# NevVerVer/DBS-Gym

Measured on AMD Instinct MI355X. Metric: env steps/sec (whole node), N=1024 osc x 4096 envs per GPU, higher is better.
Workload: dtype f32 (bf16x3-split products, f32 accumulate)

## Files before the change

### dbs-gym_amd/abi.py

```python
from __future__ import annotations

import ctypes
import os
from ctypes import POINTER, c_double, c_float, c_int, c_int32, c_int64, c_uint8, c_void_p

KURA_ABI_VERSION = 2
KURA_S_MAX = 32
KURA_MAX_BINS = 32
KURA_NSTATS = 8

KURA_F_MAX_STEPS = 1
KURA_F_NONFINITE = 2
KURA_F_GRID = 8
KURA_F_BARRIER = 16
KURA_F_BOUNDS = 32
FLAG_NAMES = {
    KURA_F_MAX_STEPS: "The maximum number of solver steps was reached",
    KURA_F_NONFINITE: "non-finite (NaN/Inf) state or RHS",
    KURA_F_GRID: "save grid outside [2, KURA_S_MAX] samples",
    KURA_F_BARRIER: "split-group barrier timed out",
    KURA_F_BOUNDS: "device access outside its buffer (KURA_DEBUG build)",
}

KURA_REC_NAIVE = 0
# ... 79 lines not shown
    "kura_create": (c_int, [POINTER(KuraConfig), c_int, POINTER(c_void_p)]),
    "kura_destroy": (c_int, [c_void_p]),
    "kura_last_error": (ctypes.c_char_p, []),
    "kura_abi_version": (c_int, []),
    "kura_set_coupling": (c_int, [c_void_p, c_void_p]),
    "kura_set_env_params": (c_int, [c_void_p, c_int, c_int, c_void_p, c_void_p, c_void_p]),
    "kura_set_spectral": (c_int, [c_void_p, c_void_p, c_void_p]),
    "kura_reset": (c_int, [c_void_p, c_void_p, c_void_p, c_void_p, c_void_p]),
    "kura_step": (c_int, [c_void_p, c_void_p, c_void_p, c_void_p, c_void_p, c_void_p, c_void_p, c_void_p,
                          c_void_p]),
    "kura_reward": (c_int, [c_void_p, c_int, c_void_p, c_void_p, c_void_p, c_int, c_void_p]),
    "kura_reward_n": (c_int, [c_void_p, c_int, c_void_p, c_int64, c_int64, c_int, c_void_p, c_void_p, c_int,
                              c_void_p, c_void_p, c_void_p]),
    "kura_get_state": (c_int, [c_void_p, c_void_p, c_void_p, c_void_p, c_void_p, c_void_p]),
    "kura_set_state": (c_int, [c_void_p, c_void_p, c_void_p, c_void_p, c_void_p, c_void_p]),
    "kura_get_spec": (c_int, [c_void_p, c_void_p]),
    "kura_set_spec": (c_int, [c_void_p, c_void_p]),
    "kura_set_env_gain": (c_int, [c_void_p, c_int, c_int, c_void_p]),
    "kura_psd_bbpow": (c_int, [c_void_p, c_void_p, c_void_p, c_int64, c_int, c_double, c_double, c_double, c_void_p,
                               c_void_p]),
    "kura_episode_bbpow": (c_int, [c_void_p, c_void_p, c_double, c_double, c_double, c_void_p, c_void_p]),
    "kura_envelope_stats": (c_int, [c_void_p, c_void_p, c_void_p, c_int64, c_int, c_void_p, c_void_p]),
    "kura_episode_envelope_stats": (c_int, [c_void_p, c_void_p, c_void_p, c_void_p]),
    "kura_get_stats": (c_int, [c_void_p, c_void_p, c_int]),
    "kura_get_env_flags": (c_int, [c_void_p, c_void_p, c_void_p]),
    "kura_set_row_capture": (c_int, [c_void_p, c_void_p]),
    "kura_set_transient_capture": (c_int, [c_void_p, c_void_p]),
    "kura_set_transient_rows": (c_int, [c_void_p, c_void_p]),
    "kura_transient_len": (c_int, [c_void_p]),
    "kura_get_stamps": (c_int, [c_void_p, c_void_p]),
    "kura_selftest_math": (c_int, [c_void_p, c_void_p, c_void_p, c_int]),
    "kura_selftest_gemm": (c_int, [c_void_p, c_void_p, c_void_p, c_int]),
    "kura_selftest_coupling": (c_int, [c_void_p, c_void_p, c_void_p, c_int, c_int]),
}

PKG_DIR = os.path.dirname(os.path.abspath(__file__))
LIB_PATH = os.path.join(PKG_DIR, "csrc", "libkura.so")

_lib = None


def load_library(path: str | None = None) -> ctypes.CDLL:
    global _lib
    if _lib is not None and path is None:
        return _lib
    p = path or os.environ.get("KURA_LIB") or LIB_PATH
    if not os.path.exists(p):
        raise RuntimeError(
            f"libkura.so not found at {p}: build it with `python -c 'import __graft_entry__ as g; g.build()'` "
            "(the HIP library is the only implementation of the step path; there is no CPU fallback)")
    lib = ctypes.CDLL(p)
    for name, (res, args) in _SYMBOLS.items():
        fn = getattr(lib, name)
        fn.restype = res
        fn.argtypes = args
    for name, (res, args) in _DEBUG_SYMBOLS.items():
        if hasattr(lib, name):
            fn = getattr(lib, name)
            fn.restype = res
            fn.argtypes = args
    if lib.kura_abi_version() != KURA_ABI_VERSION:
        raise RuntimeError("libkura ABI version mismatch")
    if path is None:
        _lib = lib
    return lib

# ... 38 lines not shown
```

### dbs-gym_amd/csrc/kura_capi.inc

```
#include <stdarg.h>
#include <stdlib.h>
#include <stdio.h>
#include <string.h>

#include <algorithm>
#include <string>
#include <unordered_map>
#include <utility>
#include <vector>

#include "kura_r2.h"

namespace {

thread_local char g_err[512] = "";

int set_err(int code, const char* fmt, ...) {
    va_list ap;
    va_start(ap, fmt);
    vsnprintf(g_err, sizeof(g_err), fmt, ap);
    va_end(ap);
    return code;
}

// ... 101 lines not shown

static void fill_params(KuraHandle* h) {
    const KuraConfig& c = h->cfg;
    DevParams& p = h->p;
    p.N = c.n_osc;
    p.B = c.n_envs;
    p.W = c.window;
    p.n_elec = c.n_elec;
    p.n_rec = c.n_rec;
    p.rec_kernel = c.rec_kernel;
    p.reward_kind = c.reward_kind;
    p.episode_steps = c.episode_steps;
    p.max_steps = c.max_steps;
    p.n_bins = c.n_bins;
    p.padlen = c.padlen;
    for (int i = 0; i < KURA_MAX_BINS; ++i) p.bins[i] = c.bins[i];
    p.dt = c.dt;
    p.width = c.width;
    p.pause = c.pause;
    p.transient_len = c.transient_len;
    p.act_lo = c.act_lo;
    p.act_hi = c.act_hi;
    p.dbs_lo = c.dbs_lo;
    p.dbs_hi = c.dbs_hi;
    for (int i = 0; i < 5; ++i) { p.bw_b[i] = c.bw_b[i]; p.bw_a[i] = c.bw_a[i]; }
    for (int i = 0; i < 4; ++i) p.bw_zi[i] = c.bw_zi[i];
    p.rtol = c.rtol;
    p.atol = c.atol;
    p.kn = c.kn;
    p.dt0 = c.dt0;
    p.alpha_sw = h->alpha_sw;
    p.alpha_dd = h->alpha_dd;
    p.alpha_dd_bytes = (unsigned)(h->alpha_dd_cap * sizeof(float));
    p.omega = h->omega;
    p.kn_env = h->kn_env;
    p.g_stim = h->g_stim;
    p.g_rec = h->g_rec;
    p.ctab = h->ctab;
    p.stab = h->stab;
    p.y = h->y;
    p.t = h->t;
    p.step = h->step;
    p.ring = h->ring;
    p.wpos = h->wpos;
    p.R = h->R;
    p.pulse = h->pulse;
    p.r2c = h->r2c;
    p.spec = h->spec;
    p.stats = h->stats;
    p.stamps = h->stamps;
    p.npart = h->xl ? c.n_osc / (h->tpw * 256) : 1;
    p.npairs = h->ngroups * p.npart;
    p.xg = h->xg;
    p.xred = h->xred;
    p.xredd = h->xredd;
    p.gcnt = h->gcnt;
    p.episode_cap = c.episode_cap;
    p.ep_lfp = h->ep_lfp;
    p.ep_len = h->ep_len;
    p.eflags = h->eflags;
    p.rows = nullptr;
    p.lfp_tr = nullptr;
    p.rows_tr = nullptr;
    p.n_tr = (int)ceil((c.transient_len - 0.0) / c.dt);
    p.gemm_dump = nullptr;
    p.gemm_dump_n = 0;
// ... 12 lines not shown
}

static uint16_t bf16_rne(float f) {
    uint32_t u;
    memcpy(&u, &f, 4);
    return (uint16_t)((u + 0x7fffu + ((u >> 16) & 1u)) >> 16);
}
static float bf16_f(uint16_t h) {
    const uint32_t u = (uint32_t)h << 16;
    float f;
    memcpy(&f, &u, 4);
    return f;
}
static void split_fragment(const float* alpha, int N, int jt, int b, uint16_t* f) {
    for (int lane = 0; lane < 64; ++lane)
        for (int i = 0; i < 8; ++i) {
            const int col = 32 * jt + (lane & 31);
            const int k = 16 * b + 8 * (i / 4) + 2 * (i % 4) + (lane >> 5);
            const float a = alpha[(size_t)col * N + k];
            const uint16_t h1 = bf16_rne(a);
            const float r1 = a - bf16_f(h1);
            const uint16_t h2 = bf16_rne(r1);
            const uint16_t h3 = bf16_rne(r1 - bf16_f(h2));
            const uint16_t hp[3] = {h1, h2, h3};
            for (int p = 0; p < 3; ++p) f[(p * 64 + lane) * 8 + i] = hp[p];
        }
}
static void split_alpha(const float* alpha, uint16_t* sp, int N) {
    const int NB = N / 16;
    for (int jt = 0; jt < N / 32; ++jt)
        for (int b = 0; b < NB; ++b) split_fragment(alpha, N, jt, b, sp + ((size_t)jt * NB + b) * 3 * 64 * 8);
}

static bool presplit_image(int N, bool sp, int tpw) {
    return sp && (N <= XL_NL || tpw > KURA_XL_SP_STAGED_MAXTPW);
}
static uint64_t fnv1a64(const void* p, size_t n) {
    const unsigned char* c = static_cast<const unsigned char*>(p);
    uint64_t h = 1469598103934665603ull;
    for (size_t i = 0; i < n; ++i) h = (h ^ c[i]) * 1099511628211ull;
    return h;
}
static std::vector<float> split_alpha_dedup(const float* alpha, int N, int* nfrag = nullptr) {
    const int NB = N / 16, NT = N / 32;
    const size_t FU16 = 3 * 64 * 8;
    const size_t MAPF = (size_t)NT * NB;
    std::vector<uint16_t> frags;
    std::vector<int32_t> map(MAPF);
    std::unordered_multimap<uint64_t, int> seen;
    std::vector<uint16_t> f(FU16);
    int n = 0;
    for (int jt = 0; jt < NT; ++jt)
        for (int b = 0; b < NB; ++b) {
            split_fragment(alpha, N, jt, b, f.data());
            const uint64_t key = fnv1a64(f.data(), FU16 * 2);
            int id = -1;
            for (auto r = seen.equal_range(key); r.first != r.second; ++r.first)
                if (!memcmp(frags.data() + (size_t)r.first->second * FU16, f.data(), FU16 * 2)) {
                    id = r.first->second;
                    break;
                }
            if (id < 0) {
                id = n++;
                seen.emplace(key, id);
                frags.insert(frags.end(), f.begin(), f.end());
            }
// ... 203 lines not shown
                    nb < 1)
                    rc = set_err(KURA_E_UNSUPPORTED, "split-group kernel does not fit a CU (occupancy %d)", nb);
            }
        }
    }
    if (rc) {
        int keep = rc;
        kura_destroy(h);
        return keep;
    }
    fill_params(h);
    *out = h;
    return KURA_OK;
}

int kura_destroy(KuraHandle* h) {
    if (!h) return KURA_OK;
    (void)hipSetDevice(h->device);
    void* ptrs[] = {h->alpha_sw, h->alpha_dd, h->omega, h->kn_env, h->g_stim, h->g_rec, h->ctab, h->stab, h->y, h->t, h->step,
                    h->ring, h->wpos, h->R, h->pulse, h->r2c, h->spec, h->stats, h->stamps,
                    h->xg, h->xred, h->xredd, h->gcnt, h->ep_lfp, h->ep_len, h->met_scratch,
                    h->eflags};
    for (void* q : ptrs)
        if (q) (void)hipFree(q);
    for (auto& kv : h->r2c_len) (void)hipFree(kv.second);
    delete h;
    return KURA_OK;
}

int kura_set_coupling(KuraHandle* h, const float* alpha) {
    if (!h || !alpha) return set_err(KURA_E_INVALID, "null argument");
    HIP_TRY(hipSetDevice(h->device));
    const int N = h->cfg.n_osc;
    const std::vector<float> sw = coupling_image(alpha, N, h->sp, h->tpw);
    if (sw.size() > h->alpha_cap) {
        HIP_TRY(hipDeviceSynchronize());
        HIP_TRY(hipFree(h->alpha_sw));
        h->alpha_sw = nullptr;
        h->alpha_cap = 0;
        if (int rc = dalloc(&h->alpha_sw, sw.size())) return rc;
        h->alpha_cap = sw.size();
        h->p.alpha_sw = h->alpha_sw;
    }
    HIP_TRY(hipMemcpy(h->alpha_sw, sw.data(), sw.size() * sizeof(float), hipMemcpyHostToDevice));
    if (h->sp && !h->xl) {
        const std::vector<float> dd = split_alpha_dedup(alpha, N);
        if (dd.size() > h->alpha_dd_cap) {
            HIP_TRY(hipDeviceSynchronize());
            if (h->alpha_dd) HIP_TRY(hipFree(h->alpha_dd));
            h->alpha_dd = nullptr;
            h->alpha_dd_cap = 0;
            if (int rc = dalloc(&h->alpha_dd, dd.size())) return rc;
            h->alpha_dd_cap = dd.size();
            h->p.alpha_dd = h->alpha_dd;
            h->p.alpha_dd_bytes = (unsigned)(dd.size() * sizeof(float));
        }
        HIP_TRY(hipMemcpy(h->alpha_dd, dd.data(), dd.size() * sizeof(float), hipMemcpyHostToDevice));
    }
    h->have_coupling = true;
    return KURA_OK;
}

int kura_set_env_params(KuraHandle* h, int env0, int n, const float* omega, const double* g_stim,
                        const double* g_rec) {
    if (!h) return set_err(KURA_E_INVALID, "null handle");
    if (env0 < 0 || n < 0 || env0 + n > h->B) return set_err(KURA_E_INVALID, "env range [%d,%d) outside [0,%d)", env0, env0 + n, h->B);
    HIP_TRY(hipSetDevice(h->device));
    const size_t N = h->cfg.n_osc;
    if (omega)
        HIP_TRY(hipMemcpy(h->omega + (size_t)env0 * N, omega, (size_t)n * N * sizeof(float), hipMemcpyHostToDevice));
    if (g_stim)
        HIP_TRY(hipMemcpy(h->g_stim + (size_t)env0 * h->cfg.n_elec * N, g_stim,
                          (size_t)n * h->cfg.n_elec * N * sizeof(double), hipMemcpyHostToDevice));
    if (g_rec && h->cfg.n_rec > 0) {
        std::vector<double> G((size_t)n * N);
        const int nr = h->cfg.n_rec;
        for (int b = 0; b < n; ++b)
            for (size_t i = 0; i < N; ++i) {
                double acc = g_rec[((size_t)b * nr) * N + i];
                for (int r = 1; r < nr; ++r) acc = acc + g_rec[((size_t)b * nr + r) * N + i];
                G[(size_t)b * N + i] = acc;
            }
        HIP_TRY(hipMemcpy(h->g_rec + (size_t)env0 * N, G.data(), G.size() * sizeof(double), hipMemcpyHostToDevice));
    }
    if (omega && g_stim) h->have_params = true;
    return KURA_OK;
}

int kura_set_env_gain(KuraHandle* h, int env0, int n, const float* kn) {
    if (!h || !kn) return set_err(KURA_E_INVALID, "null argument");
    if (env0 < 0 || n < 0 || env0 + n > h->B) return set_err(KURA_E_INVALID, "env range [%d,%d) outside [0,%d)", env0, env0 + n, h->B);
    for (int b = 0; b < n; ++b)
        if (!(kn[b] == kn[b])) return set_err(KURA_E_INVALID, "kn[%d] is nan", env0 + b);
// ... 401 lines not shown
    for (int i = 0; i < n && i < KURA_NSTATS; ++i) out[i] = (int64_t)v[i];
    return KURA_OK;
}

int kura_get_stamps(KuraHandle* h, uint64_t* out ) {
    if (!h || !out) return set_err(KURA_E_INVALID, "null argument");
    HIP_TRY(hipSetDevice(h->device));
    HIP_TRY(hipDeviceSynchronize());
    HIP_TRY(hipMemcpy(out, h->stamps, NWAVES * KURA_NSTAMP * sizeof(uint64_t), hipMemcpyDeviceToHost));
    HIP_TRY(hipMemset(h->stamps, 0, NWAVES * KURA_NSTAMP * sizeof(uint64_t)));
    return KURA_OK;
}

int kura_selftest_math(const float* x, const float* y, float* out, int n) {
    if (n <= 0 || !x || !y || !out) return set_err(KURA_E_INVALID, "bad args");
    float *dx = nullptr, *dy = nullptr, *dout = nullptr;
    int rc = dalloc(&dx, n);
    rc = rc ? rc : dalloc(&dy, n);
    rc = rc ? rc : dalloc(&dout, (size_t)n * KURA_SELFTEST_MATH_W);
    if (!rc) {
        (void)hipMemcpy(dx, x, n * sizeof(float), hipMemcpyHostToDevice);
        (void)hipMemcpy(dy, y, n * sizeof(float), hipMemcpyHostToDevice);
        hipLaunchKernelGGL(kura_selftest_math_kernel, dim3((n + 255) / 256), dim3(256), 0, 0, dx, dy, dout, n);
        hipError_t e = hipDeviceSynchronize();
        if (e != hipSuccess) rc = set_err(KURA_E_HIP, "selftest_math: %s", hipGetErrorString(e));
        else (void)hipMemcpy(out, dout, (size_t)n * KURA_SELFTEST_MATH_W * sizeof(float), hipMemcpyDeviceToHost);
    }
    (void)hipFree(dx);
    (void)hipFree(dy);
    (void)hipFree(dout);
    return rc;
}

int kura_selftest_coupling(const float* X , const float* alpha , float* Y , int N,
                           int coupling) {
    if (N != 256 && N != 512 && N != 1024) return set_err(KURA_E_UNSUPPORTED, "N=%d", N);
    if (coupling != KURA_COUPLING_AUTO && coupling != KURA_COUPLING_F32 && coupling != KURA_COUPLING_BF16X3)
        return set_err(KURA_E_INVALID, "coupling=%d", coupling);
    const bool sp = coupling != KURA_COUPLING_F32;
    const std::vector<float> sw = coupling_image(alpha, N, sp, N / 256);
    float *dX = nullptr, *dA = nullptr, *dY = nullptr;
    int rc = dalloc(&dX, (size_t)32 * N);
    rc = rc ? rc : dalloc(&dA, sw.size());
    rc = rc ? rc : dalloc(&dY, (size_t)32 * N);
    const size_t lds = (size_t)xs_floats(N) * sizeof(float);
    const void* k = selftest_gemm_kernel(N / 256, sp);
    if (!rc && hipFuncSetAttribute(k, hipFuncAttributeMaxDynamicSharedMemorySize, (int)lds) != hipSuccess)
        rc = set_err(KURA_E_HIP, "selftest_gemm: LDS attribute");
    if (!rc) {
        (void)hipMemcpy(dX, X, (size_t)32 * N * sizeof(float), hipMemcpyHostToDevice);
        (void)hipMemcpy(dA, sw.data(), sw.size() * sizeof(float), hipMemcpyHostToDevice);
        void* argv[] = {(void*)&dX, (void*)&dA, (void*)&dY, (void*)&N};
        hipError_t e = hipLaunchKernel(k, dim3(1), dim3(NTHREADS), argv, lds, 0);
        if (e == hipSuccess) e = hipDeviceSynchronize();
        if (e != hipSuccess) rc = set_err(KURA_E_HIP, "selftest_gemm: %s", hipGetErrorString(e));
        else (void)hipMemcpy(Y, dY, (size_t)32 * N * sizeof(float), hipMemcpyDeviceToHost);
    }
    (void)hipFree(dX);
    (void)hipFree(dA);
    (void)hipFree(dY);
    return rc;
}

int kura_selftest_gemm(const float* X, const float* alpha, float* Y, int N) {
    return kura_selftest_coupling(X, alpha, Y, N, KURA_COUPLING_F32);
}

}
```

### dbs-gym_amd/csrc/kura_kernels.hip

```cpp
#include <hip/hip_runtime.h>
#include <stdint.h>

#include "../../include/kura.h"
#include "kura_detmath.h"

#pragma clang fp contract(off)

#define E_WG 16
#define NWAVES 8
#define NTHREADS (NWAVES * 64)
#define ENVS_PER_WAVE (E_WG / NWAVES)

typedef float floatx4 __attribute__((ext_vector_type(4)));
typedef float floatx16 __attribute__((ext_vector_type(16)));
typedef unsigned int v4u32 __attribute__((ext_vector_type(4)));

#define KF(x) ((float)(x))
__device__ constexpr float kA[7][6] = {
    {0, 0, 0, 0, 0, 0},
    {KF(1.0 / 5.0), 0, 0, 0, 0, 0},
    {KF(3.0 / 40.0), KF(9.0 / 40.0), 0, 0, 0, 0},
    {KF(44.0 / 45.0), KF(-56.0 / 15.0), KF(32.0 / 9.0), 0, 0, 0},
    {KF(19372.0 / 6561.0), KF(-25360.0 / 2187.0), KF(64448.0 / 6561.0), KF(-212.0 / 729.0), 0, 0},
    {KF(9017.0 / 3168.0), KF(-355.0 / 33.0), KF(46732.0 / 5247.0), KF(49.0 / 176.0), KF(-5103.0 / 18656.0), 0},
    {KF(35.0 / 384.0), 0, KF(500.0 / 1113.0), KF(125.0 / 192.0), KF(-2187.0 / 6784.0), KF(11.0 / 84.0)}};
__device__ constexpr float kE[7] = {KF(35.0 / 384.0 - 1951.0 / 21600.0), 0,
                                    KF(500.0 / 1113.0 - 22642.0 / 50085.0), KF(125.0 / 192.0 - 451.0 / 720.0),
                                    KF(-2187.0 / 6784.0 + 12231.0 / 42400.0), KF(11.0 / 84.0 - 649.0 / 6300.0),
                                    KF(-1.0 / 60.0)};
__device__ constexpr float kM[7] = {KF(6025192743.0 / 30085553152.0 / 2.0), 0,
                                    KF(51252292925.0 / 65400821598.0 / 2.0),
                                    KF(-2691868925.0 / 45128329728.0 / 2.0),
                                    KF(187940372067.0 / 1594534317056.0 / 2.0),
                                    KF(-1776094331.0 / 19743644256.0 / 2.0), KF(11237099.0 / 235043384.0 / 2.0)};
#undef KF

struct DevParams {
    int N, B, W, n_elec, n_rec, rec_kernel, reward_kind, episode_steps, max_steps, n_bins, padlen;
    int bins[KURA_MAX_BINS];
    double dt, width, pause, transient_len, act_lo, act_hi, dbs_lo, dbs_hi;
    double bw_b[5], bw_a[5], bw_zi[4];
    float rtol, atol, kn, dt0;
    const float* alpha_sw;
    const float* alpha_dd;
    unsigned alpha_dd_bytes;
    const float* omega;
    const float* kn_env;
    const double* g_stim;
    const double* g_rec;
    const double* ctab;
    const double* stab;
    float* y;
    double* t;
    int* step;
    double* ring;
    int* wpos;
    float* R;
    float* pulse;
    const double* r2c;
    double* spec;
    unsigned long long* stats;
    unsigned long long* stamps;
    int npart;
    int npairs;
    float* xg;
    float* xred;
    double* xredd;
    unsigned* gcnt;
    int episode_cap;
    float* ep_lfp;
    int* ep_len;
    int* eflags;
    float* rows;
    double* lfp_tr;
    float* rows_tr;
    int n_tr;
    float* gemm_dump;
    int gemm_dump_n;
// ... 249 lines not shown
            acc[t] = __builtin_amdgcn_mfma_f32_32x32x16_bf16(x2, a1[d][t], acc[t], 0, 0, 0);
            acc[t] = __builtin_amdgcn_mfma_f32_32x32x16_bf16(x3, a1[d][t], acc[t], 0, 0, 0);
            acc[t] = __builtin_amdgcn_mfma_f32_32x32x16_bf16(x1, a2[d][t], acc[t], 0, 0, 0);
            acc[t] = __builtin_amdgcn_mfma_f32_32x32x16_bf16(x2, a2[d][t], acc[t], 0, 0, 0);
            acc[t] = __builtin_amdgcn_mfma_f32_32x32x16_bf16(x1, a3[d][t], acc[t], 0, 0, 0);
#else
            acc[t] = __builtin_amdgcn_mfma_f32_32x32x16_bf16(x1, a1[d][t], acc[t], 0, 0, 0);
            acc[t] = __builtin_amdgcn_mfma_f32_32x32x16_bf16(x1, a2[d][t], acc[t], 0, 0, 0);
            acc[t] = __builtin_amdgcn_mfma_f32_32x32x16_bf16(x2, a1[d][t], acc[t], 0, 0, 0);
            acc[t] = __builtin_amdgcn_mfma_f32_32x32x16_bf16(x1, a3[d][t], acc[t], 0, 0, 0);
            acc[t] = __builtin_amdgcn_mfma_f32_32x32x16_bf16(x2, a2[d][t], acc[t], 0, 0, 0);
            acc[t] = __builtin_amdgcn_mfma_f32_32x32x16_bf16(x3, a1[d][t], acc[t], 0, 0, 0);
#endif
#if KURA_EXP_ALPHA == 3
            gth(t, bn, a1[d][t], a2[d][t], a3[d][t]);
#elif KURA_EXP_ALPHA != 2
            a1[d][t] = ld(t, bn, 0);
            a2[d][t] = ld(t, bn, 1);
            a3[d][t] = ld(t, bn, 2);
#else
            (void)bn;
#endif
        }
        __builtin_amdgcn_sched_barrier(0);
    };
    static_assert(NB % 2 == 0, "two-block ring");
#pragma unroll 1
    for (int b = 0; b < NB; b += 2) {
        blk(b, 0);
        blk(b + 1, 1);
    }
}

template <int TPW>
__device__ __forceinline__ void coupling_gemm_f32(const float* __restrict__ Xs, const float* __restrict__ alpha_sw,
                                                  floatx16 (&acc)[TPW], unsigned long long* dbg = nullptr) {
    (void)dbg;
    constexpr int N = TPW * 32 * NWAVES;
    constexpr int NK8 = N / 8;
    constexpr int TSTRIDE = NK8 * 64;
    int lane;
    asm volatile("v_mbcnt_lo_u32_b32 %0, -1, 0\n\tv_mbcnt_hi_u32_b32 %0, -1, %0" : "=v"(lane));
    const int wave = __builtin_amdgcn_readfirstlane(threadIdx.x >> 6);
#pragma unroll
    for (int t = 0; t < TPW; ++t)
#pragma unroll
        for (int r = 0; r < 16; ++r) acc[t][r] = 0.0f;
    const floatx4* xs4 = reinterpret_cast<const floatx4*>(Xs + (lane >> 5) * XS_HALF + (lane & 31) * 4);
    const float* au = uniform_ptr(alpha_sw);
    const __amdgpu_buffer_rsrc_t rs = __builtin_amdgcn_make_buffer_rsrc(
        (void*)(au + (size_t)wave * TPW * TSTRIDE * 4), 0, TPW * TSTRIDE * 16, 0x00020000);
    auto ld = [&](int t, int k) -> floatx4 {
        KDBG_CHECK(dbg, k >= 0 && k < NK8 && (lane + k * 64) * 16 + t * TSTRIDE * 16 + 16 <=
                                                                        TPW * TSTRIDE * 16);
        return __builtin_bit_cast(floatx4, __builtin_amdgcn_raw_buffer_load_b128(rs, (lane + k * 64) * 16,
                                                                                 t * TSTRIDE * 16, 0));
    };
    floatx4 b0[TPW], b1[TPW];
#pragma unroll
    for (int t = 0; t < TPW; ++t) {
        b0[t] = ld(t, 0);
        b1[t] = ld(t, 1);
    }
#pragma unroll 1
    for (int kb = 0; kb < NK8; kb += 2) {
        floatx4 a = xs4[kb * (XS_BLOCK / 4)];
// ... 54 lines not shown
        }
#pragma unroll
    for (int t = 0; t < TPW; ++t) om[t] = off(t, 2 < NB ? 2 : NB - 1);
    auto blk = [&](int b, int d) __attribute__((always_inline)) {
        bf16x8 x1, x2, x3;
        split_bf16x3(xs4[(2 * b) * (XS_BLOCK / 4)], xs4[(2 * b + 1) * (XS_BLOCK / 4)], x1, x2, x3);
        const int bn3 = b + 3 < NB ? b + 3 : NB - 1;
#pragma unroll
        for (int t = 0; t < TPW; ++t) {
            acc[t] = __builtin_amdgcn_mfma_f32_32x32x16_bf16(x1, a1[d][t], acc[t], 0, 0, 0);
            acc[t] = __builtin_amdgcn_mfma_f32_32x32x16_bf16(x1, a2[d][t], acc[t], 0, 0, 0);
            acc[t] = __builtin_amdgcn_mfma_f32_32x32x16_bf16(x2, a1[d][t], acc[t], 0, 0, 0);
            acc[t] = __builtin_amdgcn_mfma_f32_32x32x16_bf16(x1, a3[d][t], acc[t], 0, 0, 0);
            acc[t] = __builtin_amdgcn_mfma_f32_32x32x16_bf16(x2, a2[d][t], acc[t], 0, 0, 0);
            acc[t] = __builtin_amdgcn_mfma_f32_32x32x16_bf16(x3, a1[d][t], acc[t], 0, 0, 0);
            const int o = om[t];
            a1[d][t] = ld(o, 0);
            a2[d][t] = ld(o, 1);
            a3[d][t] = ld(o, 2);
            om[t] = off(t, bn3);
        }
        __builtin_amdgcn_sched_barrier(0);
    };
    static_assert(NB % 2 == 0, "two-block ring");
#pragma unroll 1
    for (int b = 0; b < NB; b += 2) {
        blk(b, 0);
        blk(b + 1, 1);
    }
}

template <int TPW, bool SP>
__device__ __forceinline__ void coupling_gemm(const float* __restrict__ Xs, const float* __restrict__ alpha_sw,
                                              floatx16 (&acc)[TPW], unsigned long long* dbg = nullptr) {
    if constexpr (SP)
        coupling_gemm_bf16x3<TPW>(Xs, alpha_sw, acc, dbg);
    else
        coupling_gemm_f32<TPW>(Xs, alpha_sw, acc, dbg);
}

#ifndef KURA_RESET_DEDUP
#define KURA_RESET_DEDUP 1
#endif


__device__ __forceinline__ void lds_barrier() {
    asm volatile("" ::: "memory");
    __builtin_amdgcn_fence(__ATOMIC_RELEASE, "workgroup", "local");
    __builtin_amdgcn_s_barrier();
    __builtin_amdgcn_fence(__ATOMIC_ACQUIRE, "workgroup", "local");
    asm volatile("" ::: "memory");
}

template <int TPW>
__device__ __forceinline__ void coupling_gemm_xl(const float* __restrict__ xg, const float* __restrict__ alpha_sw,
                                                 float* Xs, int NG, int col0, floatx16 (&acc)[TPW] STAMP_PARAMS) {
    NG = __builtin_amdgcn_readfirstlane(NG);
    col0 = __builtin_amdgcn_readfirstlane(col0);
    xg = uniform_ptr(xg);
    const int NK8 = NG / 8;
    const int TSTRIDE = NK8 * 64;
    const int nchunk = NG / XL_KC;
    int lane;
    asm volatile("v_mbcnt_lo_u32_b32 %0, -1, 0\n\tv_mbcnt_hi_u32_b32 %0, -1, %0" : "=v"(lane));
    const int wave = __builtin_amdgcn_readfirstlane(threadIdx.x >> 6);
#pragma unroll
    for (int t = 0; t < TPW; ++t)
#pragma unroll
        for (int r = 0; r < 16; ++r) acc[t][r] = 0.0f;
    const float* au = uniform_ptr(alpha_sw);
// ... 1484 lines not shown
    }
    STAMP_DECL
    long long nrhs = 0;
    int s = 0;
    stage_input<TPW>(ws, Xs, 0 STAMP_ARGS);
    STAMP(0);
    for (;;) {
        floatx16 acc[TPW];
#ifdef KURA_EXP_NO_B1
        if (XL || s == 0 || s == 1) lds_barrier();
#else
        lds_barrier();
#endif
        STAMP(1);
        const float* xown = nullptr;
        if constexpr (XL) {
            const float* xgrp = uniform_ptr(group_publish_x<TPW>(p, pt, Xs));
            xown = xgrp + (size_t)__builtin_amdgcn_readfirstlane(pt.part) * xl_img(TPW);
            STAMP(16);
            if constexpr (SP) {
#ifdef KURA_DEBUG
                unsigned long long* dbg = uniform_ptr(p.stats);
#else
                unsigned long long* dbg = nullptr;
#endif
                if constexpr (TPW > KURA_XL_SP_STAGED_MAXTPW)
                    coupling_gemm_xl_bf16x3_kb<TPW>(xgrp, p.alpha_sw, Xs, NG, col0, acc, dbg STAMP_ARGS);
                else
                    coupling_gemm_xl_bf16x3<TPW>(xgrp, p.alpha_sw, Xs, NG, col0, acc, dbg STAMP_ARGS);
            } else
                coupling_gemm_xl<TPW>(xgrp, p.alpha_sw, Xs, NG, col0, acc STAMP_ARGS);
        } else {
#ifdef KURA_DEBUG
            coupling_gemm<TPW, SP>(Xs, p.alpha_sw, acc, uniform_ptr(p.stats));
            if (p.gemm_dump && blockIdx.x == 0 && nrhs < p.gemm_dump_n) {
                float* d = p.gemm_dump + (size_t)nrhs * 2 * 32 * N;
                for (int idx = tid; idx < 32 * N; idx += NTHREADS) d[idx] = Xs[xs_idx(idx / N, idx % N)];
#pragma unroll
                for (int t = 0; t < TPW; ++t)
#pragma unroll
                    for (int q = 0; q < 16; ++q)
                        d[32 * N + (size_t)((q & 3) + 8 * (q >> 2) + 4 * (lane >> 5)) * N + 32 * (wave * TPW + t) +
                          (lane & 31)] = acc[t][q];
            }
#else
#if KURA_RESET_DEDUP
            if constexpr (SP && RS)
                coupling_gemm_bf16x3_dd<TPW>(Xs, p.alpha_dd, p.alpha_dd_bytes, acc);
            else
#endif
                coupling_gemm<TPW, SP>(Xs, p.alpha_sw, acc);
#endif
        }
        STAMP(2);
#ifdef KURA_FUSED_ERR
        if (s == 6) coupling_epilogue_err<TPW, XL>(p, ws, Xs, xown, acc, pulse_on);
        else
#endif
            coupling_epilogue<TPW, XL>(p, ws, Xs, xown, acc, s, pulse_on);
        STAMP(3);
#ifdef KURA_EXP_NO_B2
        if (XL || s == 0 || s == 6) lds_barrier();
#else
        lds_barrier();
#endif
        STAMP(4);
        ++nrhs;
        if (s > 0 && s < 6) {
            ++s;
            stage_input<TPW>(ws, Xs, s STAMP_ARGS);
            STAMP(0);
            continue;
        }
        int any;
        if (s == 6) {
            any = post_step<TPW, XL, RS>(p, ws, env_base, pt STAMP_ARGS);
            STAMP(10);
        } else {
            if (tid < E_WG && s_ctl[tid].active) s_ctl[tid].h = s_ctl[tid].tnext - s_ctl[tid].tprev;
            any = 0;
#pragma unroll
            for (int e = 0; e < E_WG; ++e) any |= __builtin_amdgcn_readfirstlane(s_ctl[e].active);
            lds_barrier();
            STAMP(6);
// ... 535 lines not shown
        if (p.reward_kind == KURA_R_BBPOW_THR) {
            r = -(1e4 * bb > 20.0 ? 5.0 : 0.0) - au;
        } else {
            r = -(1e4 * bb) - 1e-2 * au;
        }
    }
    if (lane == 0) out[j] = r;
}

#include "kura_fft.inc"

#define KURA_SELFTEST_MATH_W 10
__global__ void kura_selftest_math_kernel(const float* x, const float* y, float* out, int n) {
    const int i = blockIdx.x * blockDim.x + threadIdx.x;
    if (i >= n) return;
    float* o = out + (size_t)i * KURA_SELFTEST_MATH_W;
    float s, c;
    kdm_sincosf(x[i], &s, &c);
    o[0] = s;
    o[1] = c;
    o[2] = kdm_fmod2pi(x[i]);
    o[3] = kdm_inv_fifth_root(fabsf(y[i]));
    o[4] = sqrtf(fabsf(x[i]));
    o[5] = x[i] / y[i];
    o[6] = (float)((double)x[i] / (double)y[i]);
    o[7] = (float)ceil((double)x[i] / 0.05);
    kdm_sincos_fmod2pi(x[i], &s, &c);
    o[8] = s;
    o[9] = c;
}

template <int TPW, bool SP>
__global__ __launch_bounds__(NTHREADS) void kura_selftest_gemm_kernel(const float* X, const float* alpha_sw,
                                                                       float* Y, int N) {
    extern __shared__ float Xs[];
    for (int idx = threadIdx.x; idx < 32 * N; idx += blockDim.x) {
        const int r = idx / N, k = idx % N;
        Xs[xs_idx(r, k)] = X[idx];
    }
    __syncthreads();
    floatx16 acc[TPW];
    coupling_gemm<TPW, SP>(Xs, alpha_sw, acc);
    const int lane = threadIdx.x & 63, wave = threadIdx.x >> 6;
#pragma unroll
    for (int t = 0; t < TPW; ++t)
#pragma unroll
        for (int q = 0; q < 16; ++q) {
            const int row = (q & 3) + 8 * (q >> 2) + 4 * (lane >> 5);
            const int col = 32 * (wave * TPW + t) + (lane & 31);
            Y[(size_t)row * N + col] = acc[t][q];
        }
}

#include "kura_capi.inc"
```

### dbs-gym_amd/sim.py

```python
from __future__ import annotations

import ctypes

import numpy as np
import torch

from . import abi
from . import spectral
from .abi import KURA_S_MAX, KuraConfig, KuraSolverError, check, ptr


def auto_part_osc(n_osc: int, n_envs: int, n_cu: int = 256) -> int:
    if n_osc <= 1024:
        return 0
    groups = -(-n_envs // 16)
    for part in (1024, 512, 256):
        if n_osc % part == 0 and groups * (n_osc // part) >= n_cu:
            return part
    return 256 if n_osc % 256 == 0 else 1024


def make_config(params: dict, n_envs: int, reward_func: str | None = None, max_steps: int = 4096,
                episode_cap: int = 0, part_osc: int = 0, coupling: str = "auto") -> KuraConfig:
    p = params
# ... 57 lines not shown

class KuraSim:

    def __init__(self, cfg: KuraConfig, device: torch.device | str | int = 0, lib_path: str | None = None):
        if not torch.cuda.is_available():
            raise RuntimeError("KuraSim needs a ROCm GPU (torch.cuda.is_available() is False); "
                               "there is no CPU implementation of the step path")
        self.lib = abi.load_library(lib_path)
        self.cfg = cfg
        self.device = torch.device("cuda", torch.device(device).index if not isinstance(device, int) else device)
        if self.device.index is None:
            self.device = torch.device("cuda", 0)
        self.B, self.N, self.W = cfg.n_envs, cfg.n_osc, cfg.window
        h = ctypes.c_void_p()
        with torch.cuda.device(self.device):
            check(self.lib, self.lib.kura_create(ctypes.byref(cfg), self.device.index, ctypes.byref(h)), "kura_create")
        self._h = h
        dev = self.device
        B = self.B
        self.obs = torch.zeros((B, self.W), dtype=torch.float32, device=dev)
        self.reward = torch.zeros(B, dtype=torch.float64, device=dev)
        self.done = torch.zeros(B, dtype=torch.uint8, device=dev)
        self.lfp_true = torch.zeros((B, KURA_S_MAX), dtype=torch.float32, device=dev)
        self.lfp_rec = torch.zeros((B, KURA_S_MAX), dtype=torch.float64, device=dev)
        self.nsamp = torch.zeros(B, dtype=torch.int32, device=dev)
        self.flags = torch.zeros(B, dtype=torch.int32, device=dev)

    def set_coupling(self, alpha: np.ndarray) -> None:
        a = np.ascontiguousarray(alpha, dtype=np.float32)
        if a.shape != (self.N, self.N):
            raise ValueError(f"alpha shape {a.shape} != ({self.N}, {self.N})")
        check(self.lib, self.lib.kura_set_coupling(self._h, a.ctypes.data), "kura_set_coupling")

    def set_env_params(self, omega, g_stim, g_rec=None, env0: int = 0) -> None:
        w = np.ascontiguousarray(omega, dtype=np.float32)
        n = w.shape[0]
        gs = np.ascontiguousarray(g_stim, dtype=np.float64)
        gr = None if g_rec is None else np.ascontiguousarray(g_rec, dtype=np.float64)
        check(self.lib, self.lib.kura_set_env_params(self._h, env0, n, w.ctypes.data, gs.ctypes.data,
                                                     None if gr is None else gr.ctypes.data),
              "kura_set_env_params")

    def set_env_gain(self, kn, env0: int = 0) -> None:
        k = np.ascontiguousarray(kn, dtype=np.float32).reshape(-1)
        check(self.lib, self.lib.kura_set_env_gain(self._h, env0, len(k), k.ctypes.data), "kura_set_env_gain")

    def set_spectral(self, cos_tab, sin_tab) -> None:
        c = np.ascontiguousarray(cos_tab, dtype=np.float64)
        s = np.ascontiguousarray(sin_tab, dtype=np.float64)
        check(self.lib, self.lib.kura_set_spectral(self._h, c.ctypes.data, s.ctypes.data), "kura_set_spectral")

    def _stream(self):
        return ctypes.c_void_p(torch.cuda.current_stream(self.device).cuda_stream)

    def reset(self, theta0: torch.Tensor, mask: torch.Tensor | None = None, check_errors: bool = False):
        th = theta0.to(self.device, torch.float32).contiguous()
        if th.shape != (self.B, self.N):
            raise ValueError("theta0 must be (B, N)")
        m = None if mask is None else mask.to(self.device, torch.uint8).contiguous()
        with torch.cuda.device(self.device):
            check(self.lib, self.lib.kura_reset(self._h, ptr(m), ptr(th), ptr(self.obs), self._stream()),
                  "kura_reset")
            check(self.lib, self.lib.kura_get_env_flags(self._h, ptr(self.flags), self._stream()),
                  "kura_get_env_flags")
        self._keep = (th, m)
        if check_errors:
# ... 181 lines not shown
```

### include/kura.h

```cpp
#ifndef KURA_H
#define KURA_H

#include <stdint.h>

#ifdef __cplusplus
extern "C" {
#endif

#define KURA_ABI_VERSION 2
#define KURA_S_MAX 32
#define KURA_MAX_BINS 32

enum {
    KURA_OK = 0,
    KURA_E_INVALID = -1,
    KURA_E_HIP = -2,
    KURA_E_NOMEM = -3,
    KURA_E_UNSUPPORTED = -4,
    KURA_E_STATE = -5
};

enum {
    KURA_F_MAX_STEPS = 1,
    KURA_F_NONFINITE = 2,
// ... 24 lines not shown
    int32_t episode_cap;
    int32_t part_osc;
    int32_t coupling;
    int32_t reserved_i[1];
    double dt;
    double width;
    double pause;
    double transient_len;
    double act_lo, act_hi;
    double dbs_lo, dbs_hi;
    double bw_b[5];
    double bw_a[5];
    double bw_zi[4];
    double reserved_d[4];
    float rtol, atol;
    float kn;
    float dt0;
    float reserved_f[4];
} KuraConfig;

static inline int kura_coupling_of(const struct KuraConfig* c) {
    if (c->coupling == KURA_COUPLING_AUTO) return KURA_COUPLING_BF16X3;
    return c->coupling;
}

typedef struct KuraHandle KuraHandle;

int kura_create(const KuraConfig* cfg, int device, KuraHandle** out);
int kura_destroy(KuraHandle* h);
const char* kura_last_error(void);
int kura_abi_version(void);

int kura_set_coupling(KuraHandle* h, const float* alpha );
int kura_set_env_params(KuraHandle* h, int env0, int n,
                        const float* omega,
                        const double* g_stim,
                        const double* g_rec);
int kura_psd_bbpow(KuraHandle* h, const float* sig, const int32_t* len, int64_t ld, int n, double psd_dt,
                   double beta_a, double beta_b, double* out, void* stream);
int kura_episode_bbpow(KuraHandle* h, const uint8_t* mask, double psd_dt, double beta_a, double beta_b,
                       double* out, void* stream);
int kura_envelope_stats(KuraHandle* h, const float* sig, const int32_t* len, int64_t ld, int n, double* out,
                        void* stream);
int kura_episode_envelope_stats(KuraHandle* h, const uint8_t* mask, double* out, void* stream);
int kura_set_env_gain(KuraHandle* h, int env0, int n, const float* kn);
int kura_set_spectral(KuraHandle* h, const double* cos_tab, const double* sin_tab );

int kura_reset(KuraHandle* h, const uint8_t* mask ,
               const float* theta0 ,
               float* obs , void* stream);
int kura_step(KuraHandle* h, const float* action ,
              float* obs,
              double* reward,
              uint8_t* done,
              float* lfp_true,
              double* lfp_rec,
              int32_t* nsamp,
              void* stream);
int kura_reward(KuraHandle* h, int kind, const double* window , const float* u0 ,
                double* reward , int n, void* stream);
int kura_reward_n(KuraHandle* h, int kind, const double* x , int64_t len, int64_t ld, int n,
                  const double* cos_tab, const double* sin_tab, int n_bins, const double* u0 ,
                  double* reward , void* stream);

int kura_get_state(KuraHandle* h, float* y , double* t , int32_t* step ,
                   double* ring , int32_t* wpos );
int kura_set_state(KuraHandle* h, const float* y, const double* t, const int32_t* step,
                   const double* ring, const int32_t* wpos);
int kura_get_spec(KuraHandle* h, double* out);
int kura_set_spec(KuraHandle* h, const double* in);
#ifdef KURA_DEBUG
int kura_debug_read_workspace(KuraHandle* h, float* out, int64_t n);
int kura_debug_gemm_dump(KuraHandle* h, float* dev_buf, int n);
#endif
int kura_set_row_capture(KuraHandle* h, float* rows_dev);

int kura_set_transient_capture(KuraHandle* h, double* lfp_dev);

int kura_set_transient_rows(KuraHandle* h, float* rows_dev);
int kura_transient_len(KuraHandle* h);

int kura_get_env_flags(KuraHandle* h, int32_t* out_dev, void* stream);

#define KURA_NSTATS 8
int kura_get_stats(KuraHandle* h, int64_t* out, int n);

int kura_selftest_math(const float* x, const float* y, float* out, int n);
int kura_selftest_gemm(const float* X, const float* alpha, float* Y, int N);
int kura_selftest_coupling(const float* X, const float* alpha, float* Y, int N, int coupling);
int kura_get_stamps(KuraHandle* h, uint64_t* out);

#ifdef __cplusplus
}
#endif
#endif
```

Baseline: 1.357 million.

## Reuse shifted alpha fragments in bf16x3 coupling GEMM when coupling is shift-invariant

At set-coupling time the host checks whether the pre-split alpha image for N=1024 is shift-invariant, meaning tile jt, block b equals tile jt-1, block b-2. If so, a flag routes the TPW=4 bf16x3 GEMM to a new kernel. That kernel keeps a rotating register ring of fragments so each loaded alpha fragment serves all four tiles, cutting global or buffer loads of alpha per step. The check is exact and an env var can disable it, so non-matching couplings fall back to the old path. The cost is a new specialised code path with tricky index arithmetic that only fires for structured (e.g. circulant or ring) coupling matrices.

```diff
diff --git a/dbs-gym_amd/abi.py b/dbs-gym_amd/abi.py
--- a/dbs-gym_amd/abi.py
+++ b/dbs-gym_amd/abi.py
@@ -135,6 +135,9 @@
     "kura_selftest_math": (c_int, [c_void_p, c_void_p, c_void_p, c_int]),
     "kura_selftest_gemm": (c_int, [c_void_p, c_void_p, c_void_p, c_int]),
     "kura_selftest_coupling": (c_int, [c_void_p, c_void_p, c_void_p, c_int, c_int]),
+    "kura_selftest_alpha_reuse": (c_int, []),
+    "kura_alpha_reuse": (c_int, [c_void_p]),
+    "kura_alpha_reuse_detect": (c_int, [c_void_p, c_int]),
 }
 
 PKG_DIR = os.path.dirname(os.path.abspath(__file__))
diff --git a/dbs-gym_amd/csrc/kura_capi.inc b/dbs-gym_amd/csrc/kura_capi.inc
--- a/dbs-gym_amd/csrc/kura_capi.inc
+++ b/dbs-gym_amd/csrc/kura_capi.inc
@@ -157,6 +157,7 @@
     p.alpha_sw = h->alpha_sw;
     p.alpha_dd = h->alpha_dd;
     p.alpha_dd_bytes = (unsigned)(h->alpha_dd_cap * sizeof(float));
+    p.alpha_reuse = 0;
     p.omega = h->omega;
     p.kn_env = h->kn_env;
     p.g_stim = h->g_stim;
@@ -235,6 +236,23 @@
         for (int b = 0; b < NB; ++b) split_fragment(alpha, N, jt, b, sp + ((size_t)jt * NB + b) * 3 * 64 * 8);
 }
 
+static bool alpha_shift_reuse(const uint16_t* sp, int N) {
+    if (N != 1024) return false;
+    const int NB = N / 16;
+    const size_t FU16 = 3 * 64 * 8;
+    for (int jt = 0; jt < N / 32; ++jt)
+        for (int b = 0; b < NB; ++b) {
+            if (jt % 4 == 0 || b % 8 < 2) continue;
+            if (memcmp(sp + ((size_t)jt * NB + b) * FU16, sp + ((size_t)(jt - 1) * NB + (b - 2)) * FU16, FU16 * 2))
+                return false;
+        }
+    return true;
+}
+static bool alpha_reuse_allowed() {
+    const char* e = getenv("KURA_ALPHA_REUSE");
+    return !(e && e[0] == '0' && e[1] == 0);
+}
+
 static bool presplit_image(int N, bool sp, int tpw) {
     return sp && (N <= XL_NL || tpw > KURA_XL_SP_STAGED_MAXTPW);
 }
@@ -504,12 +522,16 @@
     if (!h || !alpha) return set_err(KURA_E_INVALID, "null argument");
     HIP_TRY(hipSetDevice(h->device));
     const int N = h->cfg.n_osc;
+    h->have_coupling = false;
+    h->p.alpha_reuse = 0;
     const std::vector<float> sw = coupling_image(alpha, N, h->sp, h->tpw);
     if (sw.size() > h->alpha_cap) {
         HIP_TRY(hipDeviceSynchronize());
-        HIP_TRY(hipFree(h->alpha_sw));
+        float* old = h->alpha_sw;
         h->alpha_sw = nullptr;
         h->alpha_cap = 0;
+        h->p.alpha_sw = nullptr;
+        HIP_TRY(hipFree(old));
         if (int rc = dalloc(&h->alpha_sw, sw.size())) return rc;
         h->alpha_cap = sw.size();
         h->p.alpha_sw = h->alpha_sw;
@@ -519,9 +541,12 @@
         const std::vector<float> dd = split_alpha_dedup(alpha, N);
         if (dd.size() > h->alpha_dd_cap) {
             HIP_TRY(hipDeviceSynchronize());
-            if (h->alpha_dd) HIP_TRY(hipFree(h->alpha_dd));
+            float* old = h->alpha_dd;
             h->alpha_dd = nullptr;
             h->alpha_dd_cap = 0;
+            h->p.alpha_dd = nullptr;
+            h->p.alpha_dd_bytes = 0;
+            if (old) HIP_TRY(hipFree(old));
             if (int rc = dalloc(&h->alpha_dd, dd.size())) return rc;
             h->alpha_dd_cap = dd.size();
             h->p.alpha_dd = h->alpha_dd;
@@ -529,8 +554,23 @@
         }
         HIP_TRY(hipMemcpy(h->alpha_dd, dd.data(), dd.size() * sizeof(float), hipMemcpyHostToDevice));
     }
+    h->p.alpha_reuse = h->sp && !h->xl && alpha_reuse_allowed() &&
+                       alpha_shift_reuse(reinterpret_cast<const uint16_t*>(sw.data()), N);
     h->have_coupling = true;
     return KURA_OK;
+}
+
+int kura_alpha_reuse(KuraHandle* h) {
+    if (!h) return set_err(KURA_E_INVALID, "null handle");
+    return h->have_coupling && h->p.alpha_reuse ? 1 : 0;
+}
+
+int kura_alpha_reuse_detect(const float* alpha, int n_osc) {
+    if (!alpha) return set_err(KURA_E_INVALID, "null argument");
+    if (n_osc != 1024) return 0;
+    std::vector<uint16_t> sp((size_t)n_osc * n_osc * 3);
+    split_alpha(alpha, sp.data(), n_osc);
+    return alpha_shift_reuse(sp.data(), n_osc) ? 1 : 0;
 }
 
 int kura_set_env_params(KuraHandle* h, int env0, int n, const float* omega, const double* g_stim,
@@ -998,6 +1038,9 @@
     return rc;
 }
 
+static int g_selftest_reuse = 0;
+int kura_selftest_alpha_reuse(void) { return g_selftest_reuse; }
+
 int kura_selftest_coupling(const float* X , const float* alpha , float* Y , int N,
                            int coupling) {
     if (N != 256 && N != 512 && N != 1024) return set_err(KURA_E_UNSUPPORTED, "N=%d", N);
@@ -1005,6 +1048,8 @@
         return set_err(KURA_E_INVALID, "coupling=%d", coupling);
     const bool sp = coupling != KURA_COUPLING_F32;
     const std::vector<float> sw = coupling_image(alpha, N, sp, N / 256);
+    int reuse = sp && alpha_reuse_allowed() && alpha_shift_reuse(reinterpret_cast<const uint16_t*>(sw.data()), N);
+    g_selftest_reuse = reuse;
     float *dX = nullptr, *dA = nullptr, *dY = nullptr;
     int rc = dalloc(&dX, (size_t)32 * N);
     rc = rc ? rc : dalloc(&dA, sw.size());
@@ -1016,7 +1061,7 @@
     if (!rc) {
         (void)hipMemcpy(dX, X, (size_t)32 * N * sizeof(float), hipMemcpyHostToDevice);
         (void)hipMemcpy(dA, sw.data(), sw.size() * sizeof(float), hipMemcpyHostToDevice);
-        void* argv[] = {(void*)&dX, (void*)&dA, (void*)&dY, (void*)&N};
+        void* argv[] = {(void*)&dX, (void*)&dA, (void*)&dY, (void*)&N, (void*)&reuse};
         hipError_t e = hipLaunchKernel(k, dim3(1), dim3(NTHREADS), argv, lds, 0);
         if (e == hipSuccess) e = hipDeviceSynchronize();
         if (e != hipSuccess) rc = set_err(KURA_E_HIP, "selftest_gemm: %s", hipGetErrorString(e));
diff --git a/dbs-gym_amd/csrc/kura_kernels.hip b/dbs-gym_amd/csrc/kura_kernels.hip
--- a/dbs-gym_amd/csrc/kura_kernels.hip
+++ b/dbs-gym_amd/csrc/kura_kernels.hip
@@ -44,6 +44,7 @@
     const float* alpha_sw;
     const float* alpha_dd;
     unsigned alpha_dd_bytes;
+    int alpha_reuse;
     const float* omega;
     const float* kn_env;
     const double* g_stim;
@@ -359,6 +360,76 @@
     }
 }
 
+__device__ __forceinline__ void coupling_gemm_bf16x3_shift(const float* __restrict__ Xs,
+                                                           const float* __restrict__ alpha_sw, floatx16 (&acc)[4],
+                                                           unsigned long long* dbg = nullptr) {
+    (void)dbg;
+    constexpr int TPW = 4;
+    constexpr int N = TPW * 32 * NWAVES;
+    constexpr int NB = N / 16;
+    constexpr int GB = 8;
+    constexpr int TSTRIDE = NB * 3 * 64 * 16;
+    static_assert(NB % GB == 0, "whole groups");
+    int lane;
+    asm volatile("v_mbcnt_lo_u32_b32 %0, -1, 0\n\tv_mbcnt_hi_u32_b32 %0, -1, %0" : "=v"(lane));
+    const int wave = __builtin_amdgcn_readfirstlane(threadIdx.x >> 6);
+#pragma unroll
+    for (int t = 0; t < TPW; ++t)
+#pragma unroll
+        for (int r = 0; r < 16; ++r) acc[t][r] = 0.0f;
+    const floatx4* xs4 = reinterpret_cast<const floatx4*>(Xs + (lane >> 5) * XS_HALF + (lane & 31) * 4);
+    const float* au = uniform_ptr(alpha_sw);
+    const __amdgpu_buffer_rsrc_t rs = __builtin_amdgcn_make_buffer_rsrc(
+        (void*)((const char*)au + (size_t)wave * TPW * TSTRIDE), 0, TPW * TSTRIDE, 0x00020000);
+    auto ld = [&](int t, int b, int p) -> bf16x8 {
+        KDBG_CHECK(dbg, t >= 0 && t < TPW && b >= 0 && b < NB &&
+                            ((b * 3 + p) * 64 + lane) * 16 + t * TSTRIDE + 16 <= TPW * TSTRIDE);
+        return __builtin_bit_cast(bf16x8, __builtin_amdgcn_raw_buffer_load_b128(rs, ((b * 3 + p) * 64 + lane) * 16,
+                                                                                 t * TSTRIDE, 0));
+    };
+    bf16x8 a1[GB], a2[GB], a3[GB];
+#pragma unroll
+    for (int d = 0; d < 2; ++d)
+#pragma unroll
+        for (int t = 0; t < TPW; ++t) {
+            const int s = (d - 2 * t + 6) & 7;
+            a1[s] = ld(t, d, 0);
+            a2[s] = ld(t, d, 1);
+            a3[s] = ld(t, d, 2);
+        }
+#pragma unroll 1
+    for (int b0 = 0; b0 < NB; b0 += GB) {
+#pragma unroll
+        for (int xb = 0; xb < GB; ++xb) {
+            bf16x8 x1, x2, x3;
+            split_bf16x3(xs4[(2 * (b0 + xb)) * (XS_BLOCK / 4)], xs4[(2 * (b0 + xb) + 1) * (XS_BLOCK / 4)], x1, x2, x3);
+#pragma unroll
+            for (int t = TPW - 1; t >= 0; --t) {
+                const int s = (xb - 2 * t + 6) & 7;
+                acc[t] = __builtin_amdgcn_mfma_f32_32x32x16_bf16(x1, a1[s], acc[t], 0, 0, 0);
+                acc[t] = __builtin_amdgcn_mfma_f32_32x32x16_bf16(x1, a2[s], acc[t], 0, 0, 0);
+                acc[t] = __builtin_amdgcn_mfma_f32_32x32x16_bf16(x2, a1[s], acc[t], 0, 0, 0);
+                acc[t] = __builtin_amdgcn_mfma_f32_32x32x16_bf16(x1, a3[s], acc[t], 0, 0, 0);
+                acc[t] = __builtin_amdgcn_mfma_f32_32x32x16_bf16(x2, a2[s], acc[t], 0, 0, 0);
+                acc[t] = __builtin_amdgcn_mfma_f32_32x32x16_bf16(x3, a1[s], acc[t], 0, 0, 0);
+                if (xb < GB - 2) {
+                    if (t == TPW - 1) {
+                        a1[s] = ld(0, b0 + xb + 2, 0);
+                        a2[s] = ld(0, b0 + xb + 2, 1);
+                        a3[s] = ld(0, b0 + xb + 2, 2);
+                    }
+                } else {
+                    const int tn = (t + 1) & 3, bn = (b0 + GB < NB ? b0 + GB : b0) + xb - (GB - 2);
+                    a1[s] = ld(tn, bn, 0);
+                    a2[s] = ld(tn, bn, 1);
+                    a3[s] = ld(tn, bn, 2);
+                }
+            }
+            __builtin_amdgcn_sched_barrier(0);
+        }
+    }
+}
+
 template <int TPW>
 __device__ __forceinline__ void coupling_gemm_f32(const float* __restrict__ Xs, const float* __restrict__ alpha_sw,
                                                   floatx16 (&acc)[TPW], unsigned long long* dbg = nullptr) {
@@ -479,10 +550,16 @@
 
 template <int TPW, bool SP>
 __device__ __forceinline__ void coupling_gemm(const float* __restrict__ Xs, const float* __restrict__ alpha_sw,
-                                              floatx16 (&acc)[TPW], unsigned long long* dbg = nullptr) {
-    if constexpr (SP)
+                                              int reuse, floatx16 (&acc)[TPW], unsigned long long* dbg = nullptr) {
+    if constexpr (SP) {
+        if constexpr (TPW == 4) {
+            if (__builtin_amdgcn_readfirstlane(reuse)) {
+                coupling_gemm_bf16x3_shift(Xs, alpha_sw, acc, dbg);
+                return;
+            }
+        }
         coupling_gemm_bf16x3<TPW>(Xs, alpha_sw, acc, dbg);
-    else
+    } else
         coupling_gemm_f32<TPW>(Xs, alpha_sw, acc, dbg);
 }
 
@@ -2033,7 +2110,7 @@
                 coupling_gemm_xl<TPW>(xgrp, p.alpha_sw, Xs, NG, col0, acc STAMP_ARGS);
         } else {
 #ifdef KURA_DEBUG
-            coupling_gemm<TPW, SP>(Xs, p.alpha_sw, acc, uniform_ptr(p.stats));
+            coupling_gemm<TPW, SP>(Xs, p.alpha_sw, p.alpha_reuse, acc, uniform_ptr(p.stats));
             if (p.gemm_dump && blockIdx.x == 0 && nrhs < p.gemm_dump_n) {
                 float* d = p.gemm_dump + (size_t)nrhs * 2 * 32 * N;
                 for (int idx = tid; idx < 32 * N; idx += NTHREADS) d[idx] = Xs[xs_idx(idx / N, idx % N)];
@@ -2050,7 +2127,7 @@
                 coupling_gemm_bf16x3_dd<TPW>(Xs, p.alpha_dd, p.alpha_dd_bytes, acc);
             else
 #endif
-                coupling_gemm<TPW, SP>(Xs, p.alpha_sw, acc);
+                coupling_gemm<TPW, SP>(Xs, p.alpha_sw, p.alpha_reuse, acc);
 #endif
         }
         STAMP(2);
@@ -2652,7 +2729,7 @@
 
 template <int TPW, bool SP>
 __global__ __launch_bounds__(NTHREADS) void kura_selftest_gemm_kernel(const float* X, const float* alpha_sw,
-                                                                       float* Y, int N) {
+                                                                       float* Y, int N, int reuse) {
     extern __shared__ float Xs[];
     for (int idx = threadIdx.x; idx < 32 * N; idx += blockDim.x) {
         const int r = idx / N, k = idx % N;
@@ -2660,7 +2737,7 @@
     }
     __syncthreads();
     floatx16 acc[TPW];
-    coupling_gemm<TPW, SP>(Xs, alpha_sw, acc);
+    coupling_gemm<TPW, SP>(Xs, alpha_sw, reuse, acc);
     const int lane = threadIdx.x & 63, wave = threadIdx.x >> 6;
 #pragma unroll
     for (int t = 0; t < TPW; ++t)
diff --git a/dbs-gym_amd/sim.py b/dbs-gym_amd/sim.py
--- a/dbs-gym_amd/sim.py
+++ b/dbs-gym_amd/sim.py
@@ -113,6 +113,11 @@
             raise ValueError(f"alpha shape {a.shape} != ({self.N}, {self.N})")
         check(self.lib, self.lib.kura_set_coupling(self._h, a.ctypes.data), "kura_set_coupling")
 
+    def alpha_reuse(self) -> bool:
+        rc = self.lib.kura_alpha_reuse(self._h)
+        check(self.lib, min(rc, 0), "kura_alpha_reuse")
+        return rc == 1
+
     def set_env_params(self, omega, g_stim, g_rec=None, env0: int = 0) -> None:
         w = np.ascontiguousarray(omega, dtype=np.float32)
         n = w.shape[0]
diff --git a/include/kura.h b/include/kura.h
--- a/include/kura.h
+++ b/include/kura.h
@@ -80,6 +80,8 @@
 int kura_abi_version(void);
 
 int kura_set_coupling(KuraHandle* h, const float* alpha );
+int kura_alpha_reuse(KuraHandle* h);
+int kura_alpha_reuse_detect(const float* alpha, int n_osc);
 int kura_set_env_params(KuraHandle* h, int env0, int n,
                         const float* omega,
                         const double* g_stim,
@@ -136,6 +138,7 @@
 int kura_selftest_math(const float* x, const float* y, float* out, int n);
 int kura_selftest_gemm(const float* X, const float* alpha, float* Y, int N);
 int kura_selftest_coupling(const float* X, const float* alpha, float* Y, int N, int coupling);
+int kura_selftest_alpha_reuse(void);
 int kura_get_stamps(KuraHandle* h, uint64_t* out);
 
 #ifdef __cplusplus
```

Measured after the change: 1.500 million (median of 6 runs). 1.11x the previous value.
